# QueensGambit/CrazyAra

Hardware: AMD Instinct MI355X
Metric: nn_evals_per_sec (higher is better)
Workload: dtype f16x3; 1 GPU; crazyhouse RISEv2 19-block (34x8x8 planes -> 5184 policy + value), batch=256, inputs resident in HBM, random-init seeded weights; batch=256, parallelism=replicas x1, precision=float16x3

## Files before the change

crazyara_amd/csrc/nn/kernels.h:

```cpp
#pragma once
#include <hip/hip_runtime.h>
#include <cstdint>

namespace cra {

typedef _Float16 half_t;

constexpr int kSquares = 64;

inline int64_t packed_weight_elems(int cout_pad, int k_total) { return int64_t(cout_pad) * k_total; }

struct ConvArgs {
    const void* x;
    const void* wpk;
    const void* wpk_lo;
    const float* bias;
    const void* resid;
    void* out;
    int batch;
    int cin;
    int cout_pad;
    int cout_real;
    int cout_ld;
    int ks;
// ... 13 lines not shown
    float pre_acc_scale;
    int dev;
    int few_boards;
    int x_ld;
};

template <typename T> void launch_conv_gemm(const ConvArgs& a, hipStream_t s);

struct BlockArgs {
    const void* x;
    void* y;
    const void* w1pk;
    const float* b1;
    const float* wdw;
    const float* b2;
    const void* w3pk;
    const void* w1pk_lo;
    const void* w3pk_lo;
    const float* b3;
    int batch, C, cop_pad, ks;
    const float* gate;
    float* pool_out;
    const float* dwpk;
};
template <typename T> void launch_block(const BlockArgs& a, hipStream_t s);
void launch_conv_gemm_x3(const ConvArgs& a, hipStream_t s);
void launch_block_x3(const BlockArgs& a, hipStream_t s);
void init_x3_kernel_attributes();
int block_x3_chunk_channels();
struct X3TowerBlock {
    const void *w1pk, *w1pk_lo, *w3pk, *w3pk_lo;
    const float* dwpk;
    const float* b3;
    const float* se_w1t;
    const float* se_w2t;
    const float* se_b;
    int cop_pad;
    int se_kind;
    float w1_inv, w3_scale, w3_inv;
    int tail;
};
static_assert(sizeof(X3TowerBlock) == 96, "the tower kernels index a device array of these");
struct X3TowerArgs {
    const float* x;
    float* y;
    const X3TowerBlock* blocks;
    int nblocks;
    int batch;
    int p8;
    int ks;
    int symmetric;
    int no_tail;
    int no_quad;
};
void launch_tower_x3(const X3TowerArgs& a, hipStream_t s);
const char* tower_x3_kernel_name(const X3TowerArgs& a);
void launch_tower_x3_tail(const X3TowerArgs& a, hipStream_t s);
void init_x3_tail_kernel_attributes();
void launch_tower_x3_quad(const X3TowerArgs& a, hipStream_t s);
void init_x3_quad_kernel_attributes();
bool block_x3w_supports(int C, int ks);
void launch_block_x3w(const BlockArgs& a, hipStream_t s);
void init_x3_wblock_kernel_attributes();
void launch_se_gate_w(const float* pool, float* gate, int kind, const float* w1t, const float* w2t, const float* b1, int batch, int C, hipStream_t s);
constexpr int kX3WSplitMaxG = 8;
struct X3WSplitArgs {
    BlockArgs blk;
    const float* x_parts;
    float* y_parts;
    int gin, G;
    int stream_in;
};
int x3w_split_chunks(int cop_pad);
int x3w_split_shares(int cop_pad, int boards, int cu_count);
void launch_block_x3w_split(const X3WSplitArgs& a, hipStream_t s);
void launch_x3w_split_finish(const float* parts, int gin, float* y, float* pool_out, int batch, int C, hipStream_t s);
void init_x3_wsplit_kernel_attributes();
struct X3WTowerBlock {
    const void *w1pk, *w1pk_lo, *w3pk, *w3pk_lo;
    const float* dwpk;
    const float* b3;
    int cop_pad, ks;
};
static_assert(sizeof(X3WTowerBlock) == 56, "tower_x3w_kernel indexes a device array of these");
struct X3WTowerArgs {
    const float* x;
    float* y;
    const X3WTowerBlock* blocks;
    int nblocks;
    const float* gate;
    float* pool_out;
    int batch, C;
};
bool tower_x3w_supports(int C, int ks);
void launch_tower_x3w(const X3WTowerArgs& a, hipStream_t s);
void init_x3_wtower_kernel_attributes();
struct NtbLayer {
    const void *wh, *wl;
    const float* bias;
};
struct NtbArgs {
    const float* x;
    float* y;
    int batch, C, D, M, H;
    NtbLayer patch, qkv, proj, projection, mhca, mhca_proj, mlp1, mlp2;
};
// ... 194 lines not shown
```

crazyara_amd/csrc/nn/precision.cpp:

```cpp
#include <cstdlib>
#include <stdexcept>

#include "rise_net.h"

namespace cra {

namespace {
constexpr bool kX3ValueHeadOneLaunch = true;
}

RiseNet::DevSwitches::DevSwitches() {
    if (const char* e = getenv("CRA_X3_CONV_DEV")) conv_dev = atoi(e);
    device_graph = getenv("CRA_DEVICE_GRAPH") != nullptr;
    lane_graph = getenv("CRA_LANE_GRAPH") != nullptr;
    lane_no_graph = getenv("CRA_LANE_NO_GRAPH") != nullptr;
    predict_copy = getenv("CRA_PREDICT_COPY") != nullptr;
    predict_zero_copy = getenv("CRA_PREDICT_ZERO_COPY") != nullptr;
    if (const char* e = getenv("CRA_LANE_LAUNCHES")) lane_launches = e[0];
    lane_sync = getenv("CRA_LANE_SYNC") != nullptr;
    if (const char* e = getenv("CRA_X3_TOWER")) x3_symmetric = e[0] == 's';
    if (const char* e = getenv("CRA_X3_SPLIT_DEV")) x3_split_dev = atoi(e);
    no_small_path = getenv("CRA_NO_SMALL_PATH") != nullptr;
    if (const char* e = getenv("CRA_SMALL_BATCH_CONV_SPLIT")) small_conv_split = atoi(e);
    tower_trace = getenv("CRA_TOWER_TRACE") != nullptr;
    x3_value_one_launch = kX3ValueHeadOneLaunch;
    if (const char* e = getenv("CRA_X3_VALUE_HEAD")) x3_value_one_launch = e[0] == 'o';
    value_head_debug = getenv("CRA_VALUE_HEAD_DEBUG") != nullptr;
    if (const char* e = getenv("CRA_VALUE_HEAD_LDS_PAD")) value_head_lds_pad = atoi(e);
    if (const char* e = getenv("CRA_VALUE_HEAD_VARIANT")) value_head_variant = atoi(e);
    x3_no_head_chain = getenv("CRA_X3_NO_HEAD_CHAIN") != nullptr;
    x3_no_tail = getenv("CRA_X3_NO_TAIL") != nullptr;
    x3_no_quad = getenv("CRA_X3_NO_QUAD") != nullptr;
    small_batch_heads_apart = getenv("CRA_SMALL_BATCH_HEADS_APART") != nullptr;
}

Precision parse_precision(const std::string& precision) {
    Precision v;
    std::string prec = precision;
    auto strip = [&](const std::string& tag) {
        if (prec.size() <= tag.size() || prec.compare(prec.size() - tag.size(), tag.size(), tag) != 0) return false;
        prec.resize(prec.size() - tag.size());
        return true;
    };
    if (strip("-3k")) v.one_launch = false;
    if (strip("-8w")) v.thin_waves = true;
    if (strip("-1wg")) v.board_split = false;
    if (strip("-1b")) v.boards_per_wg = 1;
    else if (strip("-2b")) v.boards_per_wg = 2;
    if (strip("-wtower")) v.wtower = v.wnet = v.wblock = true;
    else if (strip("-wsplit")) v.wsplit = v.wnet = v.wblock = true;
    else if (strip("-wnet")) v.wnet = v.wblock = true;
    else if (strip("-wblock")) v.wblock = true;
    if (strip("-unfused")) v.fused = v.tower = false;
    else if (strip("-perblock")) v.tower = false;
    using M = Precision::Mode;
    static const std::pair<const char*, M> kModes[] = {
        {"float16", M::Float16},   {"fp16", M::Float16},     {"half", M::Float16},      {"int8", M::Int8},
        {"fp8", M::Fp8},           {"float8", M::Fp8},       {"float32", M::Float32},   {"fp32", M::Float32},
        {"float16x3", M::Float16x3}, {"fp16x3", M::Float16x3}, {"f16x3", M::Float16x3},
        {"float16p8", M::Float16p8}, {"fp16p8", M::Float16p8}, {"f16p8", M::Float16p8}};
    for (const auto& m : kModes)
        if (prec == m.first) {
            v.mode = m.second;
            if (v.wtower && !v.x3()) throw std::invalid_argument("`-wtower` is a float16x3 kernel family (float16x3-wtower | float16p8-wtower), got '" + precision + "'");
            if (v.wtower && !v.fused) throw std::invalid_argument("`-wtower` and `-unfused` exclude each other, got '" + precision + "'");
            if (v.wsplit && !v.x3()) throw std::invalid_argument("`-wsplit` is a float16x3 kernel family (float16x3-wsplit | float16p8-wsplit), got '" + precision + "'");
            if (v.wsplit && !v.fused) throw std::invalid_argument("`-wsplit` and `-unfused` exclude each other, got '" + precision + "'");
            if (v.wsplit && !v.board_split)
                throw std::invalid_argument("`-wsplit` and `-1wg` exclude each other (several workgroups per board against one), got '" + precision + "'");
            if (v.wnet && !v.x3()) throw std::invalid_argument("`-wnet` is a float16x3 kernel family (float16x3-wnet | float16p8-wnet), got '" + precision + "'");
            if (v.wnet && !v.fused) throw std::invalid_argument("`-wnet` and `-unfused` exclude each other, got '" + precision + "'");
            if (v.wblock && !v.x3()) throw std::invalid_argument("`-wblock` is a float16x3 kernel family (float16x3-wblock | float16p8-wblock), got '" + precision + "'");
            if (v.wblock && !v.fused) throw std::invalid_argument("`-wblock` and `-unfused` exclude each other, got '" + precision + "'");
            return v;
        }
    throw std::invalid_argument("unsupported precision '" + precision + "' (float16 | float16x3 | float16p8 | float32 | fp8 | int8)");
}

}
```

crazyara_amd/csrc/nn/rise_net.h:

```cpp
#pragma once
#include <hip/hip_runtime.h>
#include <memory>
#include <string>
#include <utility>
#include <vector>

#include "board_net.h"
#include "netfile.h"

namespace cra {

uint8_t float_to_e4m3(float v);
uint8_t float_to_e5m2(float v);

struct Precision {
    enum class Mode { Float32, Float16, Float16x3, Float16p8, Fp8, Int8 };
    Mode mode = Mode::Float16;
    bool fused = true;
    bool tower = true;
    bool one_launch = true;
    bool thin_waves = false;
    bool board_split = true;
    bool wblock = false;
    bool wnet = false;
// ... 57 lines not shown
    void time_ops(int iters, float* ms);
    float time_forward(int iters);

    struct IoOverride {
        const float* planes = nullptr;
        float* value = nullptr;
        float* probs = nullptr;
        float* aux = nullptr;
    };
    bool last_submit_was_zero_copy() const { return last_zero_copy_; }

private:
    friend class ExpertSet;
    struct ForwardCall {
        int boards = 0;
        const IoOverride* io = nullptr;
        int prev_g = 1;
    };
    RiseNet(const std::string& model_path, int device_id, int batch_size, const std::string& precision, const RiseNet* parent);
    struct Impl;
    template <typename T> struct Builder;
    template <typename T> void build(const NetFile& nf);
    template <typename T> void enqueue(hipStream_t s, ForwardCall call);
    template <typename T> void launch_op(int i, hipStream_t s, ForwardCall& call);
    void launch_forward_in_stream(ForwardCall call);
    void forward_on(hipStream_t s, ForwardCall call);
    int boards_of_call(int n_valid) const;
    void capture();
    bool buffers_are_pinned(const float* in_planes, float* value, float* probs, float* aux);
    bool last_zero_copy_ = false;
    bool counted_in_flight_ = false;
    int staged_calls_left_ = 0;
    struct DevSwitches {
        int conv_dev = -1;
        bool device_graph = false;
        bool lane_graph = false;
        bool lane_no_graph = false;
        bool predict_copy = false;
        bool predict_zero_copy = false;
        char lane_launches = 0;
        bool lane_sync = false;
        bool x3_symmetric = false;
        int x3_split_dev = 0;
        bool no_small_path = false;
        int small_conv_split = 2;
        bool tower_trace = false;
        bool x3_value_one_launch;
        bool value_head_debug = false;
        int value_head_lds_pad = -1;
        int value_head_variant = 0;
        bool x3_no_head_chain = false;
        bool x3_no_tail = false;
        bool x3_no_quad = false;
        bool small_batch_heads_apart = false;
        DevSwitches();
    } dev_;
    float* value_head_dbg_ = nullptr;

    std::string model_file_path_;
    Precision prec_;
    std::vector<std::pair<float, float>> int8_calib_;
    static constexpr int kBoardSplitMaxBatch = 64;
    std::unique_ptr<RiseNet> small_;
    bool owns_stream_ = true;
    int stream_slot_ = -1;
    std::string precision_arg_;
    int cu_count_ = 256;
    int launches_ = 0;
    hipGraph_t graph_ = nullptr;
    hipGraphExec_t graph_exec_ = nullptr;
    void* d_desc_ = nullptr;
    std::unique_ptr<Impl> impl_;
};

std::string int8_calibration_path(const std::string& model_file_path);
std::vector<std::pair<float, float>> read_int8_calibration(const std::string& model_file_path);
std::string calibrate_int8(const std::string& model_path, int device_id, const float* planes_host, int n_boards);
std::vector<float> default_calibration_planes(int channels, int version, int* n_boards);

}
```

crazyara_amd/csrc/nn/rise_net_build.hip:

```cpp
#include <algorithm>
#include <cmath>
#include <cstring>
#include <type_traits>

#include "../chess/planes_host.h"
#include "pack.h"
#include "rise_net_impl.h"

namespace cra {

namespace {
enum class Family {
    Tower,
    X3Tower,
    X3Split,
    Fused,
    WBlock,
    WSplit,
    WTower,
    Layers,
    Transformer,
    WNtb
};
struct BlockPlan {
// ... 675 lines not shown
    prod_op = int(im.ops.size());
    im.ops.push_back(op);
    tower_blocks.clear();
    tower_gate = nullptr;
    std::swap(cur, nxt);
}

template <typename T> void RiseNet::Builder<T>::flush_x3_run() {
    if (x3_blocks.empty()) return;
    if (x3_split && x3_run_ks == 3) {
        if (!split_parts[0])
            for (auto& q : split_parts) q = static_cast<float*>(im.dalloc(size_t(B) * kSplitMaxG * kSquares * C * sizeof(float)));
        const int max_g = std::max(1, std::min(int(kSplitMaxG), net.cu_count_ / B));
        const int nb = int(x3_blocks.size());
        int gin = 1;
        for (int k = 0; k < nb; ++k) {
            Op op;
            op.kind = OpKind::BlockX3Split;
            op.xs.blk = x3_blocks[k];
            op.xs.x_parts = k == 0 ? reinterpret_cast<const float*>(cur) : split_parts[k % 2];
            op.xs.y_parts = split_parts[(k + 1) % 2];
            op.xs.gin = gin;
            op.xs.batch = B;
            op.xs.G = std::min(max_g, x3_blocks[k].cop_pad / block_x3_chunk_channels());
            op.xs.dev = dev.x3_split_dev;
            if (k > 0 && x3_blocks[k].se_kind != 0 && !(dev.x3_split_dev & 8)) {
                float* pools = static_cast<float*>(im.dalloc(size_t(B) * kSplitMaxG * C * sizeof(float)));
                im.ops.back().xs.pool_out = pools;
                op.xs.pool_in = pools;
            }
            gin = op.xs.G;
            im.ops.push_back(op);
        }
        Op fin;
        fin.kind = OpKind::X3SplitFinish;
        fin.xs.x_parts = split_parts[nb % 2];
        fin.xs.gin = gin;
        fin.xs.batch = B;
        fin.xs_y = reinterpret_cast<float*>(nxt);
        im.ops.push_back(fin);
    } else {
        Op op;
        op.kind = OpKind::TowerX3;
        op.tx.x = reinterpret_cast<const float*>(cur);
        op.tx.y = reinterpret_cast<float*>(nxt);
        op.tx.blocks = im.upload(x3_blocks);
        op.tx.nblocks = int(x3_blocks.size());
        op.tx.batch = B;
        op.tx.p8 = prec.p8() ? 1 : 0;
        op.tx.ks = x3_run_ks;
        op.tx.symmetric = dev.x3_symmetric ? 1 : 0;
        op.tx.no_tail = dev.x3_no_tail ? 1 : 0;
        op.tx.no_quad = dev.x3_no_quad ? 1 : 0;
        im.ops.push_back(op);
    }
    x3_blocks.clear();
    prod_op = -1;
    std::swap(cur, nxt);
}

template <typename T> void RiseNet::Builder<T>::one_launch_head() {
    const Folded fv = fold_bn(nf, "value_head.body.0", "value_head.body.1");
    const HeadStreams hs = pack_head(fold_bn(nf, "policy_head.body.0", "policy_head.body.1"), fold_bn(nf, "policy_head.body.3", ""), fv, C, cv, cp);
    Op op;
    op.kind = OpKind::Head;
    HeadArgs& h = op.hd;
    h.x = cur;
    h.logits = net.d_logits_;
    h.probs = net.d_probs_;
    h.value = net.d_value_;
    h.aux = net.d_aux_;
    h.s1 = im.upload(hs.s1);
    h.b1 = im.upload(hs.b1);
    h.s2 = im.upload(hs.s2);
    h.s1_wave_frags = 9 * 16 + 16 + 16;
    h.s2_wave_frags = 18 * 3 + 9;
    h.vconv_bias = im.upload_d2f(fv.b, 8);
    h.cp = cp;
    h.batch = B;
    if (dev.tower_trace) h.trace = static_cast<unsigned long long*>(im.dalloc(64 * sizeof(unsigned long long)));
    const int nfl = kSquares * cv;
    if (wdl) {
        h.fc1_w = im.upload(pack_value_wdl(nf, nfl, 512));
        const float* bw = nf.get("value_head.body_wdl.0.bias").data;
        h.wdl_b[0] = bw[0]; h.wdl_b[1] = bw[1]; h.wdl_b[2] = bw[2];
        h.wdl_b[3] = nf.get("value_head.body_plys.0.bias").data[0];
        h.wdlp = 1;
        macs += 4.0 * nfl;
    } else {
        const TensorView& w2 = nf.get("value_head.body_final.2.weight");
        const float* bb = nf.get("value_head.body_final.0.bias").data;
        h.fc1_w = im.upload(pack_value_fc1_threads(nf, nfl, fc));
        h.fc1_b = im.upload(std::vector<float>(bb, bb + fc));
        h.fc2_w = im.upload(std::vector<float>(w2.data, w2.data + fc));
        h.fc2_b = nf.get("value_head.body_final.2.bias").data[0];
        macs += double(nfl) * fc + fc;
    }
    macs += double(kSquares) * 9 * (double(C) * C + double(C) * cp) + double(kSquares) * C * cv;
    im.ops.push_back(op);
}

template <typename T> void RiseNet::Builder<T>::policy_head() {
    const bool head_chain = prec.p8() && policy_map && C == 256 && round_up(cp, 16) <= 128 && !x3_split;
    const bool head_chain_x3 = prec.x3() && !prec.p8() && prec.fused && policy_map && C == 256 && round_up(cp, 16) <= 128 && !x3_split &&
                               !dev.x3_no_head_chain;
    if (head_chain || head_chain_x3) {
// ... 207 lines not shown
```

crazyara_amd/csrc/nn/x3.hip:

```cpp
#include "kernels.h"
#include "device_utils.h"
#include "value_head_body.h"
#include "x3_device.h"

#include <algorithm>
#include <cstdlib>
#include <stdexcept>
#include <type_traits>

#ifndef X3_SGB_VALU
#define X3_SGB_VALU 10
#endif

namespace cra {

namespace {

typedef int i32x4_x3 __attribute__((ext_vector_type(4)));
typedef int i32x8_x3 __attribute__((ext_vector_type(8)));
__device__ __forceinline__ uint32_t x3_high_bytes(uint32_t p01, uint32_t p23) {
    return __builtin_amdgcn_perm(p23, p01, 0x07050301u);
}
__device__ __forceinline__ void split4_b8(const float (&v)[4], half4& hi, uint32_t& h8, uint32_t& l8) {
    uint32_t h[2], l[2];
// ... 1943 lines not shown
            *reinterpret_cast<f32x4*>(yb + size_t(x3_square(t * 16 + l15)) * C + (w * NJ + j) * 16 + lg * 4) = accX[j][t];
}

void init_x3_kernel_attributes() {
    (void)hipFuncSetAttribute(reinterpret_cast<const void*>(&block_x3_kernel), hipFuncAttributeMaxDynamicSharedMemorySize, int(X3Block::lds_bytes));
    (void)hipFuncSetAttribute(reinterpret_cast<const void*>(&tower_x3_kernel), hipFuncAttributeMaxDynamicSharedMemorySize, int(X3Block::lds_bytes));
    (void)hipFuncSetAttribute(reinterpret_cast<const void*>(&block_x3_split_kernel), hipFuncAttributeMaxDynamicSharedMemorySize, int(X3Block::lds_bytes));
    (void)hipFuncSetAttribute(reinterpret_cast<const void*>(&tower_x3_roles_kernel<3>), hipFuncAttributeMaxDynamicSharedMemorySize, int(X3Block::lds_bytes));
    (void)hipFuncSetAttribute(reinterpret_cast<const void*>(&tower_x3_roles_kernel<5>), hipFuncAttributeMaxDynamicSharedMemorySize, int(X3Block::lds_bytes + 8192));
    init_x3_tail_kernel_attributes();
    init_x3_quad_kernel_attributes();
    (void)hipFuncSetAttribute(reinterpret_cast<const void*>(&tower_p8_kernel<3>), hipFuncAttributeMaxDynamicSharedMemorySize, int(X3Block::lds_bytes));
    (void)hipFuncSetAttribute(reinterpret_cast<const void*>(&tower_p8_kernel<5>), hipFuncAttributeMaxDynamicSharedMemorySize, int(X3Block::lds_bytes + 8192));
    (void)hipFuncSetAttribute(reinterpret_cast<const void*>(&conv3x3_x3_chain_kernel), hipFuncAttributeMaxDynamicSharedMemorySize, int(ConvX3::lds_bytes));
    const int conv_p8_lds = int(ConvP8::lds_bytes);
    (void)hipFuncSetAttribute(reinterpret_cast<const void*>(&conv3x3_p8_chain_kernel), hipFuncAttributeMaxDynamicSharedMemorySize, conv_p8_lds);
    (void)hipFuncSetAttribute(reinterpret_cast<const void*>(&conv3x3_p8_kernel<2, 8>), hipFuncAttributeMaxDynamicSharedMemorySize, conv_p8_lds);
    (void)hipFuncSetAttribute(reinterpret_cast<const void*>(&conv3x3_p8_kernel<1, 8>), hipFuncAttributeMaxDynamicSharedMemorySize, conv_p8_lds);
}
int block_x3_chunk_channels() { return X3Block::CK; }

void launch_block_x3(const BlockArgs& a, hipStream_t s) {
    hipLaunchKernelGGL(block_x3_kernel, dim3(a.batch), dim3(X3Block::NTHR), X3Block::lds_bytes, s, a);
}
void launch_block_x3_split(const X3SplitArgs& a, hipStream_t s) {
    const int n = a.blk.cop_pad / X3Block::CK;
    if (a.G < 1 || a.G > n || a.G > 16 || a.gin < 1 || a.gin > 16) throw std::invalid_argument("block_x3_split: 1 <= G <= min(chunks, 16), 1 <= gin <= 16");
    hipLaunchKernelGGL(block_x3_split_kernel, dim3(8 * a.G * ((a.batch + 7) / 8)), dim3(X3Block::NTHR), X3Block::lds_bytes, s, a);
}
void launch_x3_split_finish(const float* parts, int gin, float* y, int batch, hipStream_t s) {
    const int n4 = batch * 64 * X3Block::C / 4;
    hipLaunchKernelGGL(x3_split_finish_kernel, dim3(std::min(1024, (n4 + 255) / 256)), dim3(256), 0, s, parts, gin, y, batch);
}
namespace {
enum class X3TowerKernel { P8_5, P8_3, Quad3, Tail5, Tail3, Roles5, Roles3, Symmetric };
X3TowerKernel pick_tower_x3(const X3TowerArgs& a) {
    const bool symmetric = a.symmetric != 0;
    if (a.p8) {
        if (symmetric) throw std::invalid_argument("Precision float16p8 runs the two-role tower only");
        return a.ks == 5 ? X3TowerKernel::P8_5 : X3TowerKernel::P8_3;
    }
    if (!symmetric && !a.no_tail) {
        if (a.ks == 5) return X3TowerKernel::Tail5;
        return a.no_quad ? X3TowerKernel::Tail3 : X3TowerKernel::Quad3;
    }
    if (a.ks == 5) return X3TowerKernel::Roles5;
    return symmetric ? X3TowerKernel::Symmetric : X3TowerKernel::Roles3;
}
}
const char* tower_x3_kernel_name(const X3TowerArgs& a) {
    switch (pick_tower_x3(a)) {
        case X3TowerKernel::P8_5: return "tower_p8_kernel<5>";
        case X3TowerKernel::P8_3: return "tower_p8_kernel<3>";
        case X3TowerKernel::Quad3: return "tower_x3_quad_kernel<3>";
        case X3TowerKernel::Tail5: return "tower_x3_tail_kernel<5>";
        case X3TowerKernel::Tail3: return "tower_x3_tail_kernel<3>";
        case X3TowerKernel::Roles5: return "tower_x3_roles_kernel<5>";
        case X3TowerKernel::Roles3: return "tower_x3_roles_kernel<3>";
        case X3TowerKernel::Symmetric: return "tower_x3_kernel";
    }
    return "?";
}
void launch_tower_x3(const X3TowerArgs& a, hipStream_t s) {
    switch (pick_tower_x3(a)) {
        case X3TowerKernel::P8_5: hipLaunchKernelGGL(tower_p8_kernel<5>, dim3(a.batch), dim3(X3Block::NTHR), X3Block::lds_bytes + 8192, s, a); break;
        case X3TowerKernel::P8_3: hipLaunchKernelGGL(tower_p8_kernel<3>, dim3(a.batch), dim3(X3Block::NTHR), X3Block::lds_bytes, s, a); break;
        case X3TowerKernel::Quad3: launch_tower_x3_quad(a, s); break;
        case X3TowerKernel::Tail5:
        case X3TowerKernel::Tail3: launch_tower_x3_tail(a, s); break;
        case X3TowerKernel::Roles5: hipLaunchKernelGGL(tower_x3_roles_kernel<5>, dim3(a.batch), dim3(X3Block::NTHR), X3Block::lds_bytes + 8192, s, a); break;
        case X3TowerKernel::Roles3: hipLaunchKernelGGL(tower_x3_roles_kernel<3>, dim3(a.batch), dim3(X3Block::NTHR), X3Block::lds_bytes, s, a); break;
        case X3TowerKernel::Symmetric: hipLaunchKernelGGL(tower_x3_kernel, dim3(a.batch), dim3(X3Block::NTHR), X3Block::lds_bytes, s, a); break;
    }
}

}
```

crazyara_amd/csrc/nn/x3_quad.cpp:

```cpp
#include "x3_device.h"
#include "x3_quad.h"

#include <type_traits>

namespace cra {

template <int KS>
__global__ __launch_bounds__(512) void tower_x3_quad_kernel(const X3TowerArgs a) {
    static_assert(KS == 3, "depthwise 3x3 (X3DepthwiseQuad); 5x5 runs stay on tower_x3_tail_kernel");
    constexpr int REC = 256;
    using G = X3Block;
    static_assert(G::NE == 1 && G::T2BUF == 2 && G::CK == 128, "the role kernel uses the NE = 1 tile geometry (two t2 buffers of 128 channels)");
    static_assert(X3Q_T2T_HALVES <= 64 * G::TROW, "t2T of a chunk lies in the [64][TROW] tile's place");
    constexpr int C = G::C, CK = G::CK, XROW = G::XROW, TROW = G::TROW;
    extern __shared__ __attribute__((aligned(16))) char smem[];
    const X3Tiles T = x3_tiles(smem);
    const int b = blockIdx.x;
    const int tid = threadIdx.x, lane = tid & 63, l15 = lane & 15, lg = lane >> 4;
    const int wave = __builtin_amdgcn_readfirstlane(tid >> 6);
    const bool expand_role = wave < 4;
    const int w = wave & 3;
    const uint32_t lane_off = uint32_t(lane) * 16u;
    x3_stage_tile(T, a.x + size_t(b) * 64 * C, nullptr, tid);
    __syncthreads();
    constexpr int EW = 2;
    half8 e_h[EW][2], e_l[EW][2];
    bool first_chunk_requested = false;
    if (expand_role) {
    for (int blk = 0; blk < a.nblocks; ++blk) {
        const X3TowerBlock& d = a.blocks[blk];
        if (blk > 0 && d.se_kind != 0) {
            x3_se_gate_from_mean(d, reinterpret_cast<float*>(T.t2h), tid);
            __syncthreads();
            first_chunk_requested = false;
#pragma unroll
            for (int ne = 0; ne < 2; ++ne) {
#pragma unroll
                for (int q = 0; q < EW; ++q) { asm volatile("" : "=v"(e_h[q][ne])); asm volatile("" : "=v"(e_l[q][ne])); }
            }
        }
        const X3Weights W = x3_weights(d.w1pk, d.w1pk_lo, d.w3pk, d.w3pk_lo, d.dwpk, d.cop_pad);
        const int n = W.cop_pad / CK;
        const bool tail = __builtin_amdgcn_readfirstlane(d.tail) != 0;
#ifdef CRA_X3_TRACE
        const bool tracing = (b == 0 || b == 131) && blk == CRA_X3_TRACE;
        int trace_n = 0;
#endif
        {
            const X3QuadOffsets qo = x3_quad_offsets(lane);
            int sto[4];
#pragma unroll
            for (int t = 0; t < 4; ++t) sto[t] = x3q_store_offset(0, l15, lg, t);
            auto e_tile = [&](int i, int ne) { return i * (CK / 16) + (tail && i == n - 1 ? w : w * 2 + ne); };
            auto load_e = [&](auto one_c, int i, int s) {
                if constexpr (X3_ABL & 16) return;
#pragma unroll
                for (int ne = 0; ne < (decltype(one_c)::value ? 1 : 2); ++ne) {
                    const uint32_t f = uint32_t(e_tile(i, ne)) * (C / 32) + uint32_t(s);
                    e_h[s % EW][ne] = x3_frag(W.w1h, lane_off, f);
                    e_l[s % EW][ne] = x3_frag(W.w1l, lane_off, f);
                }
            };
            auto load_first_chunk = [&](const X3Weights& Wx, bool one) {
                if constexpr (X3_ABL & 16) return;
#pragma unroll
                for (int s = 0; s < EW; ++s)
#pragma unroll
                    for (int ne = 0; ne < 2; ++ne) {
                        const uint32_t f = uint32_t(one ? w : w * 2 + ne) * (C / 32) + uint32_t(s);
                        e_h[s][ne] = x3_frag(Wx.w1h, lane_off, f);
                        e_l[s][ne] = x3_frag(Wx.w1l, lane_off, f);
                    }
            };
            if constexpr (X3_ABL & 16) {
#pragma unroll
                for (int s = 0; s < EW; ++s)
#pragma unroll
                    for (int ne = 0; ne < 2; ++ne) e_h[s][ne] = e_l[s][ne] = *reinterpret_cast<const half8*>(T.xh + lane * 8);
            }
            if (!first_chunk_requested) load_first_chunk(W, tail && n == 1);
            float* const my_dws = T.dws + (w * 2) * REC;
            f32x4 accE[2][4], accD[2][4];
            X3DepthwiseQuad dw;
            auto interval = [&](auto hase_c, auto hasd_c, auto onee_c, auto oned_c, int i) {
                constexpr bool HASE = decltype(hase_c)::value, HASD = decltype(hasd_c)::value;
                constexpr bool ONEE = decltype(onee_c)::value, ONED = decltype(oned_c)::value;
                static_assert(!(ONEE && !HASE) && !(ONED && (HASE || !HASD)), "the tail chunk is expanded in interval n - 1 and runs the depthwise alone in interval n");
                constexpr int NEE = ONEE ? 1 : 2;
                half8 ring_h[4], ring_l[4];
                auto read_step = [&](int st) {
                    if constexpr (X3_ABL & 8) {
                        ring_h[st % 4] = e_h[0][0];
                        ring_l[st % 4] = e_l[0][0];
                    } else {
                        ring_h[st % 4] = *reinterpret_cast<const half8*>(T.xh + ((st & 3) * 16 + l15) * XROW + (st >> 2) * 32 + lg * 8);
                        ring_l[st % 4] = *reinterpret_cast<const half8*>(T.xl + ((st & 3) * 16 + l15) * XROW + (st >> 2) * 32 + lg * 8);
                    }
                };
                f32x4 dw_raw[NEE][REC / 256];
                if constexpr (HASE) {
// ... 47 lines not shown
                                if constexpr (X3_ABL & 64) {
                                    asm volatile("" ::"v"(h), "v"(l));
                                } else {
                                    *reinterpret_cast<half4*>(t2h + tile * 16 * X3Q_T2T_ROW + sto[t]) = h;
                                    *reinterpret_cast<half4*>(t2l + tile * 16 * X3Q_T2T_ROW + sto[t]) = l;
                                }
                            }
                        }
                    }
                    if constexpr (HASE && HASD) {
#pragma unroll
                        for (int r = 0; r < 12 * NEE; ++r) {
                            __builtin_amdgcn_sched_group_barrier(0x008, 1, 0);
                            __builtin_amdgcn_sched_group_barrier(0x002, ONEE ? 8 : 4, 0);
                        }
                    }
                    __builtin_amdgcn_sched_barrier(0);
                }
                if constexpr (HASE) {
#pragma unroll
                    for (int ne = 0; ne < NEE; ++ne)
#pragma unroll
                        for (int h2 = 0; h2 < REC / 256; ++h2) *reinterpret_cast<f32x4*>(my_dws + ne * REC + h2 * 256 + lane * 4) = dw_raw[ne][h2];
#pragma unroll
                    for (int ne = 0; ne < NEE; ++ne)
#pragma unroll
                        for (int t = 0; t < 4; ++t) accD[ne][t] = accE[ne][t];
                }
            };
            constexpr std::true_type yes{};
            constexpr std::false_type no{};
            auto run = [&](auto hase_c, auto hasd_c, auto onee_c, auto oned_c, int i) {
                const int kk = i - 1;
                X3_STAMP(0);
                interval(hase_c, hasd_c, onee_c, oned_c, i);
                X3_STAMP(3);
                if constexpr (!(X3_ABL & 32)) __syncthreads();
                X3_STAMP(4);
            };
            const int nfull = tail ? n - 1 : n;
            if (nfull == 0) run(yes, no, yes, no, 0);
            else run(yes, no, no, no, 0);
            for (int i = 1; i < nfull; ++i) run(yes, yes, no, no, i);
            if (tail) {
                if (nfull > 0) run(yes, yes, yes, no, n - 1);
                run(no, yes, no, yes, n);
            } else run(no, yes, no, no, n);
            first_chunk_requested = false;
            if (blk + 1 < a.nblocks && a.blocks[blk + 1].se_kind == 0) {
                const X3TowerBlock& dn = a.blocks[blk + 1];
                load_first_chunk(x3_weights(dn.w1pk, dn.w1pk_lo, dn.w3pk, dn.w3pk_lo, dn.dwpk, dn.cop_pad), dn.tail != 0 && dn.cop_pad == CK);
                first_chunk_requested = true;
            }
            __syncthreads();
            { const int kk = n; X3_STAMP(5); }
        }
    }
    } else {
    constexpr int NJ = 4;
    f32x4 accX[NJ][4];
    x3_stream_load<NJ>(accX, a.x + size_t(b) * 64 * C, w * NJ, l15, lg);
    for (int blk = 0; blk < a.nblocks; ++blk) {
        const X3TowerBlock& d = a.blocks[blk];
        if (blk > 0 && d.se_kind != 0) x3_stream_se<NJ>(T, d, accX, reinterpret_cast<float*>(T.t2h), w * NJ, tid);
        const X3Weights W = x3_weights(d.w1pk, d.w1pk_lo, d.w3pk, d.w3pk_lo, d.dwpk, d.cop_pad);
        const int n = W.cop_pad / CK;
        const int nslab3 = W.cop_pad >> 5;
        const bool tail = __builtin_amdgcn_readfirstlane(d.tail) != 0;
#ifdef CRA_X3_TRACE
        const bool tracing = (b == 0 || b == 131) && blk == CRA_X3_TRACE;
        int trace_n = 0;
#endif
        {
            constexpr int PW = 2;
            half8 p_h[PW][NJ], p_l[PW][NJ];
            int rdo[2][4];
#pragma unroll
            for (int hh = 0; hh < 2; ++hh)
#pragma unroll
                for (int t = 0; t < 4; ++t) rdo[hh][t] = x3q_read_offset(0, hh, t, l15, lg);
            auto load_p = [&](int k, int s2) {
                if constexpr (X3_ABL & 16) return;
#pragma unroll
                for (int j = 0; j < NJ; ++j) {
                    const uint32_t f = uint32_t(w * NJ + j) * uint32_t(nslab3) + uint32_t(k * (CK / 32) + s2);
                    p_h[s2 % PW][j] = x3_frag(W.w3h, lane_off, f);
                    p_l[s2 % PW][j] = x3_frag(W.w3l, lane_off, f);
                }
            };
            if constexpr (X3_ABL & 16) {
#pragma unroll
                for (int s2 = 0; s2 < PW; ++s2)
#pragma unroll
                    for (int j = 0; j < NJ; ++j) p_h[s2][j] = p_l[s2][j] = *reinterpret_cast<const half8*>(T.xl + lane * 8);
            }
            x3_stream_add_bias<NJ>(accX, d.b3, w * NJ, lg);
#pragma unroll
            for (int s2 = 0; s2 < PW; ++s2) load_p(0, s2);
            if constexpr (!(X3_ABL & 32)) {
                __syncthreads();
                __syncthreads();
            }
            auto project = [&](auto one_c, int kk) {
                constexpr int NS2 = decltype(one_c)::value ? CK / 64 : CK / 32;
                const half_t* const t2h = T.t2h + (kk & 1) * 64 * TROW;
                const half_t* const t2l = T.t2l + (kk & 1) * 64 * TROW;
                const half_t* rd[2][4];
#pragma unroll
                for (int hh = 0; hh < 2; ++hh)
#pragma unroll
                    for (int t = 0; t < 4; ++t) rd[hh][t] = t2h + rdo[hh][t];
                const int to_lo = int(t2l - t2h);
                X3_STAMP(8);
                half8 bh[2][4], bl[2][4];
                auto read_t2 = [&](int s2, half8 (&h)[4], half8 (&l)[4]) {
#pragma unroll
                    for (int t = 0; t < 4; ++t) {
                        if constexpr (X3_ABL & 8) {
                            h[t] = p_h[s2 % PW][0];
                            l[t] = p_l[s2 % PW][0];
                        } else {
                            h[t] = x3q_read_fragment(rd[0][t] + s2 * 32 * X3Q_T2T_ROW, rd[1][t] + s2 * 32 * X3Q_T2T_ROW);
                            l[t] = x3q_read_fragment(rd[0][t] + s2 * 32 * X3Q_T2T_ROW + to_lo, rd[1][t] + s2 * 32 * X3Q_T2T_ROW + to_lo);
                        }
                    }
                };
                read_t2(0, bh[0], bl[0]);
#pragma unroll
                for (int s2 = 0; s2 < NS2; ++s2) {
                    if (s2 + 1 < NS2) read_t2(s2 + 1, bh[(s2 + 1) & 1], bl[(s2 + 1) & 1]);
                    __builtin_amdgcn_sched_barrier(0);
#pragma unroll
                    for (int j = 0; j < NJ; ++j)
#pragma unroll
                        for (int t = 0; t < 4; ++t) x3_mfma(p_l[s2 % PW][j], bh[s2 & 1][t], accX[j][t], !(X3_ABL & 4));
#pragma unroll
                    for (int j = 0; j < NJ; ++j)
#pragma unroll
                        for (int t = 0; t < 4; ++t) x3_mfma(p_h[s2 % PW][j], bl[s2 & 1][t], accX[j][t], !(X3_ABL & 4));
#pragma unroll
                    for (int j = 0; j < NJ; ++j)
#pragma unroll
                        for (int t = 0; t < 4; ++t) x3_mfma(p_h[s2 % PW][j], bh[s2 & 1][t], accX[j][t], !(X3_ABL & 4));
                    if (s2 + PW < NS2) load_p(kk, s2 + PW);
                    else if constexpr (decltype(one_c)::value) load_p(kk, s2 + PW - NS2);
                    else load_p(kk + 1 < n ? kk + 1 : kk, s2 + PW - NS2);
                    if (s2 == 1) X3_STAMP(9);
                    __builtin_amdgcn_sched_barrier(0);
                }
                X3_STAMP(10);
            };
            const int nfull = tail ? n - 1 : n;
            for (int kk = 0; kk < nfull; ++kk) {
                project(std::false_type{}, kk);
                if (kk + 1 < n) {
                    if constexpr (!(X3_ABL & 32)) __syncthreads();
                }
                X3_STAMP(11);
            }
            if (tail) {
                const int kk = n - 1;
                project(std::true_type{}, kk);
                X3_STAMP(11);
            }
            if (blk + 1 < a.nblocks && a.blocks[blk + 1].se_kind == 0) x3_stream_write_tiles<NJ>(T, accX, w * NJ, l15, lg);
            { const int kk = n; X3_STAMP(12); }
            __syncthreads();
            { const int kk = n; X3_STAMP(13); }
        }
    }
    x3_stream_store<NJ>(accX, a.y + size_t(b) * 64 * C, w * NJ, l15, lg);
    }
}

void init_x3_quad_kernel_attributes() {
    (void)hipFuncSetAttribute(reinterpret_cast<const void*>(&tower_x3_quad_kernel<3>), hipFuncAttributeMaxDynamicSharedMemorySize, int(X3Block::lds_bytes));
}
void launch_tower_x3_quad(const X3TowerArgs& a, hipStream_t s) {
    hipLaunchKernelGGL(tower_x3_quad_kernel<3>, dim3(a.batch), dim3(X3Block::NTHR), X3Block::lds_bytes, s, a);
}

}
```

crazyara_amd/csrc/nn/x3_quad.h:

```cpp
#pragma once

namespace cra {

constexpr int x3q_row(int sq) { return ((sq >> 3) & 3) * 16 + (sq >> 5) * 8 + (sq & 7); }
constexpr int x3q_square(int row) { return ((row >> 4) + 4 * ((row >> 3) & 1)) * 8 + (row & 7); }
constexpr int x3q_lane_square(int t, int lg, int r) { return (4 * (lg >> 1) + t) * 8 + 4 * (lg & 1) + r; }

constexpr int X3Q_T2T_ROW = 64;
constexpr int X3Q_T2T_HALVES = 128 * X3Q_T2T_ROW;
constexpr int x3q_swizzle(int c) { return (c & 1) | (((c >> 2) & 1) << 1) | (((c >> 1) & 1) << 2) | (c & 8); }
constexpr int x3q_t2t_offset(int c, int row) { return c * X3Q_T2T_ROW + 4 * ((row >> 2) ^ x3q_swizzle(c & 15)) + (row & 3); }
constexpr int x3q_store_offset(int tile, int l15, int lg, int t) { return x3q_t2t_offset(tile * 16 + l15, t * 16 + 4 * lg); }
constexpr int x3q_read_offset(int s2, int hh, int t, int l15, int lg) { return x3q_t2t_offset(s2 * 32 + lg * 8 + hh * 4 + (l15 >> 2), t * 16 + 4 * (l15 & 3)); }

}

#ifdef __HIPCC__
namespace cra {
namespace {

struct X3QuadOffsets {
    int hl, hr;
    int vt, vt6;
    int vb2, vb;
    int k0, k6, k2, k8;
    int to_v, to_k;
};
__device__ __forceinline__ X3QuadOffsets x3_quad_offsets(int lane) {
    const int lg = lane >> 4;
    const bool odd = (lg & 1) != 0, hi = lg >= 2;
    X3QuadOffsets o;
    o.hl = odd ? 0 : 11 * 16;
    o.hr = odd ? 5 * 16 : 0;
    o.vt = hi ? 0 : 11 * 16;
    o.vt6 = hi ? 0 : 5 * 16;
    o.vb2 = hi ? 11 * 16 : 0;
    o.vb = hi ? 6 * 16 : 0;
    o.k0 = lg == 3 ? 0 : 11 * 16;
    o.k6 = lg == 2 ? 0 : 5 * 16;
    o.k2 = lg == 1 ? 0 : 11 * 16;
    o.k8 = lg == 0 ? 0 : 5 * 16;
    o.to_v = (lane ^ 32) * 4;
    o.to_k = (lane ^ 48) * 4;
    return o;
}

struct X3DepthwiseQuad {
    float w[11];
    float whl[3], whr[3];
    float wvt[3], wvb[3];
    float wk[4];
    float S[4][4], H[4], V[4], K;
    float outv[4][4];

    __device__ __forceinline__ void load(const float* rec, int l15, const X3QuadOffsets& o) {
        const float* p = rec + l15;
#pragma unroll
        for (int q = 0; q < 11; ++q) w[q] = p[q * 16];
#pragma unroll
        for (int d = 0; d < 3; ++d) {
            whl[d] = p[o.hl + d * 16];
            whr[d] = p[o.hr + (6 + d) * 16];
            wvt[d] = p[(d == 2 ? o.vt6 : o.vt) + 3 * d * 16];
            wvb[d] = p[(d == 0 ? o.vb2 : o.vb) + (3 * d + 2) * 16];
        }
        wk[0] = p[o.k0];
// ... 9 lines not shown
        if constexpr (X3_ABL & 1) return;
        const bool odd = (lg & 1) != 0, hi = lg >= 2;
        float sh[4];
#pragma unroll
        for (int t = 0; t < 4; ++t) {
            sh[t] = odd ? S[t][0] : S[t][3];
            H[t] = __builtin_bit_cast(float, __builtin_amdgcn_ds_swizzle(__builtin_bit_cast(int, sh[t]), 0x401f));
        }
#pragma unroll
        for (int r = 0; r < 4; ++r) {
            const float sv = hi ? S[0][r] : S[3][r];
            V[r] = __builtin_bit_cast(float, __builtin_amdgcn_ds_bpermute(o.to_v, __builtin_bit_cast(int, sv)));
        }
        const float sk = hi ? sh[0] : sh[3];
        K = __builtin_bit_cast(float, __builtin_amdgcn_ds_bpermute(o.to_k, __builtin_bit_cast(int, sk)));
    }
    template <int Y, int X, int Q> __device__ __forceinline__ float tap(float a) const {
        constexpr int DX = Q / 3, DY = Q % 3;
        if constexpr (Y >= 0 && Y < 4 && X >= 0 && X < 4) return fmaf(w[Q], S[Y][X], a);
        else if constexpr (Y >= 0 && Y < 4) return fmaf(X < 0 ? whl[DY] : whr[DY], H[Y], a);
        else if constexpr (X >= 0 && X < 4) return fmaf(Y < 0 ? wvt[DX] : wvb[DX], V[X], a);
        else return fmaf(wk[(Y < 0 ? 0 : 2) + (X < 0 ? 0 : 1)], K, a);
    }
    template <int T, int R> __device__ __forceinline__ void output() {
        if constexpr (X3_ABL & 1) {
            outv[T][R] = S[T][R];
            return;
        }
        float a = w[10];
        a = tap<T - 1, R - 1, 0>(a); a = tap<T - 1, R, 3>(a); a = tap<T - 1, R + 1, 6>(a);
        a = tap<T, R - 1, 1>(a);     a = tap<T, R, 4>(a);     a = tap<T, R + 1, 7>(a);
        a = tap<T + 1, R - 1, 2>(a); a = tap<T + 1, R, 5>(a); a = tap<T + 1, R + 1, 8>(a);
        outv[T][R] = fmaxf(a, 0.f);
    }
    template <int T> __device__ __forceinline__ void taps_rank() {
        output<T, 0>(); output<T, 1>(); output<T, 2>(); output<T, 3>();
    }
    template <int T> __device__ __forceinline__ void pin_rank() {
#pragma unroll
        for (int r = 0; r < 4; ++r) asm volatile("" : "+v"(outv[T][r]));
    }
};

typedef __fp16 x3q_f16x4 __attribute__((__vector_size__(4 * sizeof(__fp16))));
__device__ __forceinline__ half8 x3q_read_fragment(const half_t* lo4, const half_t* hi4) {
    typedef __attribute__((address_space(3))) x3q_f16x4 lds_f16x4;
    typedef uint32_t u32x2 __attribute__((ext_vector_type(2)));
    typedef uint32_t u32x4 __attribute__((ext_vector_type(4)));
    const u32x2 a = __builtin_bit_cast(u32x2, __builtin_amdgcn_ds_read_tr16_b64_v4f16((lds_f16x4*)(lo4)));
    const u32x2 b = __builtin_bit_cast(u32x2, __builtin_amdgcn_ds_read_tr16_b64_v4f16((lds_f16x4*)(hi4)));
    return __builtin_bit_cast(half8, u32x4{a.x, a.y, b.x, b.y});
}

}
}
#endif
```

Baseline: 353,600 evals/s.

## Prefetch SE gate weights early and park them in LDS for the quad tower

For squeeze-excitation blocks of kind 1, the expand-role waves now request the next block's SE FC weights during the previous block's tail. Part of the first FC matrix is parked in the xh/xl LDS tiles for the stream-role waves, and the expand role computes the FCs there directly. The stream role's SE step reads the parked weights from LDS instead of global memory, aiming to hide gate-weight load latency behind the previous block's work. The old behaviour stays behind a CRA_X3_LATE_GATE switch. This adds extra barriers, register pressure from 48 f32x4 weight registers, and reuse of LDS that must not clash with the tiles.

```diff
diff --git a/crazyara_amd/csrc/nn/kernels.h b/crazyara_amd/csrc/nn/kernels.h
--- a/crazyara_amd/csrc/nn/kernels.h
+++ b/crazyara_amd/csrc/nn/kernels.h
@@ -89,6 +89,7 @@
     int symmetric;
     int no_tail;
     int no_quad;
+    int late_gate;
 };
 void launch_tower_x3(const X3TowerArgs& a, hipStream_t s);
 const char* tower_x3_kernel_name(const X3TowerArgs& a);
diff --git a/crazyara_amd/csrc/nn/precision.cpp b/crazyara_amd/csrc/nn/precision.cpp
--- a/crazyara_amd/csrc/nn/precision.cpp
+++ b/crazyara_amd/csrc/nn/precision.cpp
@@ -31,6 +31,7 @@
     x3_no_head_chain = getenv("CRA_X3_NO_HEAD_CHAIN") != nullptr;
     x3_no_tail = getenv("CRA_X3_NO_TAIL") != nullptr;
     x3_no_quad = getenv("CRA_X3_NO_QUAD") != nullptr;
+    x3_late_gate = getenv("CRA_X3_LATE_GATE") != nullptr;
     small_batch_heads_apart = getenv("CRA_SMALL_BATCH_HEADS_APART") != nullptr;
 }
 
diff --git a/crazyara_amd/csrc/nn/rise_net.h b/crazyara_amd/csrc/nn/rise_net.h
--- a/crazyara_amd/csrc/nn/rise_net.h
+++ b/crazyara_amd/csrc/nn/rise_net.h
@@ -133,6 +133,7 @@
         bool x3_no_head_chain = false;
         bool x3_no_tail = false;
         bool x3_no_quad = false;
+        bool x3_late_gate = false;
         bool small_batch_heads_apart = false;
         DevSwitches();
     } dev_;
diff --git a/crazyara_amd/csrc/nn/rise_net_build.hip b/crazyara_amd/csrc/nn/rise_net_build.hip
--- a/crazyara_amd/csrc/nn/rise_net_build.hip
+++ b/crazyara_amd/csrc/nn/rise_net_build.hip
@@ -751,6 +751,7 @@
         op.tx.symmetric = dev.x3_symmetric ? 1 : 0;
         op.tx.no_tail = dev.x3_no_tail ? 1 : 0;
         op.tx.no_quad = dev.x3_no_quad ? 1 : 0;
+        op.tx.late_gate = dev.x3_late_gate ? 1 : 0;
         im.ops.push_back(op);
     }
     x3_blocks.clear();
diff --git a/crazyara_amd/csrc/nn/x3.hip b/crazyara_amd/csrc/nn/x3.hip
--- a/crazyara_amd/csrc/nn/x3.hip
+++ b/crazyara_amd/csrc/nn/x3.hip
@@ -2019,7 +2019,7 @@
     switch (pick_tower_x3(a)) {
         case X3TowerKernel::P8_5: return "tower_p8_kernel<5>";
         case X3TowerKernel::P8_3: return "tower_p8_kernel<3>";
-        case X3TowerKernel::Quad3: return "tower_x3_quad_kernel<3>";
+        case X3TowerKernel::Quad3: return a.late_gate ? "tower_x3_quad_kernel<3, late gate>" : "tower_x3_quad_kernel<3>";
         case X3TowerKernel::Tail5: return "tower_x3_tail_kernel<5>";
         case X3TowerKernel::Tail3: return "tower_x3_tail_kernel<3>";
         case X3TowerKernel::Roles5: return "tower_x3_roles_kernel<5>";
diff --git a/crazyara_amd/csrc/nn/x3_quad.cpp b/crazyara_amd/csrc/nn/x3_quad.cpp
--- a/crazyara_amd/csrc/nn/x3_quad.cpp
+++ b/crazyara_amd/csrc/nn/x3_quad.cpp
@@ -5,7 +5,10 @@
 
 namespace cra {
 
-template <int KS>
+static_assert(X3Q_PARK_BYTES <= int(2 * 64 * X3Block::XROW * sizeof(half_t)), "the parked gate matrix lies in xh + xl");
+constexpr int X3Q_TRACE_GATE = 13;
+
+template <int KS, bool LATE_GATE = false>
 __global__ __launch_bounds__(512) void tower_x3_quad_kernel(const X3TowerArgs a) {
     static_assert(KS == 3, "depthwise 3x3 (X3DepthwiseQuad); 5x5 runs stay on tower_x3_tail_kernel");
     constexpr int REC = 256;
@@ -27,11 +30,38 @@
     half8 e_h[EW][2], e_l[EW][2];
     bool first_chunk_requested = false;
     if (expand_role) {
+#ifdef CRA_X3_TRACE
+    int trace_n = 0;
+#endif
     for (int blk = 0; blk < a.nblocks; ++blk) {
         const X3TowerBlock& d = a.blocks[blk];
-        if (blk > 0 && d.se_kind != 0) {
+#ifdef CRA_X3_TRACE
+        const bool tracing = (b == 0 || b == 131) && blk == CRA_X3_TRACE;
+#endif
+        if (blk > 0 && d.se_kind != 0 && (LATE_GATE || d.se_kind != 1)) {
+#ifdef CRA_X3_TRACE
+            {
+                constexpr int kk = X3Q_TRACE_GATE;
+                f32x4 wa[16], wb[16];
+#pragma unroll
+                for (int i = 0; i < 16; ++i) wa[i] = reinterpret_cast<const f32x4*>(d.se_w1t)[i * 512 + tid];
+#pragma unroll
+                for (int i = 0; i < 16; ++i) wb[i] = reinterpret_cast<const f32x4*>(d.se_kind == 1 ? d.se_w2t : d.se_w1t + size_t(16) * 512 * 4)[i * 512 + tid];
+                X3_STAMP(0);
+#pragma unroll
+                for (int i = 0; i < 16; ++i) { asm volatile("s_waitcnt vmcnt(0)" : "+v"(wa[i]), "+v"(wb[i])); }
+                X3_STAMP(1);
+                __syncthreads();
+                X3_STAMP(2);
+                x3_se_fcs(d, reinterpret_cast<float*>(T.t2h), reinterpret_cast<float*>(T.t2h) + 8 * 36, reinterpret_cast<float*>(T.t2h) + 12 * 36, wa, wb, tid);
+                X3_STAMP(3);
+                __syncthreads();
+                X3_STAMP(4);
+            }
+#else
             x3_se_gate_from_mean(d, reinterpret_cast<float*>(T.t2h), tid);
             __syncthreads();
+#endif
             first_chunk_requested = false;
 #pragma unroll
             for (int ne = 0; ne < 2; ++ne) {
@@ -42,10 +72,6 @@
         const X3Weights W = x3_weights(d.w1pk, d.w1pk_lo, d.w3pk, d.w3pk_lo, d.dwpk, d.cop_pad);
         const int n = W.cop_pad / CK;
         const bool tail = __builtin_amdgcn_readfirstlane(d.tail) != 0;
-#ifdef CRA_X3_TRACE
-        const bool tracing = (b == 0 || b == 131) && blk == CRA_X3_TRACE;
-        int trace_n = 0;
-#endif
         {
             const X3QuadOffsets qo = x3_quad_offsets(lane);
             int sto[4];
@@ -199,25 +225,59 @@
                 load_first_chunk(x3_weights(dn.w1pk, dn.w1pk_lo, dn.w3pk, dn.w3pk_lo, dn.dwpk, dn.cop_pad), dn.tail != 0 && dn.cop_pad == CK);
                 first_chunk_requested = true;
             }
-            __syncthreads();
-            { const int kk = n; X3_STAMP(5); }
+            if (!LATE_GATE && blk + 1 < a.nblocks && a.blocks[blk + 1].se_kind == 1) {
+                const X3TowerBlock& dn = a.blocks[blk + 1];
+#ifdef CRA_X3_TRACE
+                const bool tracing = (b == 0 || b == 131) && blk + 1 == CRA_X3_TRACE;
+                constexpr int kk = X3Q_TRACE_GATE;
+#endif
+                f32x4 wa[16], wb[16];
+                x3q_gate_request(dn, reinterpret_cast<f32x4*>(T.xh), wa, wb, tid);
+                X3_STAMP(0);
+#ifdef CRA_X3_TRACE
+#pragma unroll
+                for (int i = 0; i < 16; ++i) { asm volatile("s_waitcnt vmcnt(0)" : "+v"(wa[i]), "+v"(wb[i])); }
+                X3_STAMP(1);
+#endif
+                __syncthreads();
+                X3_STAMP(5);
+                __syncthreads();
+                X3_STAMP(2);
+                float* const scratch = reinterpret_cast<float*>(T.t2h);
+                x3_se_fcs(dn, scratch, scratch + 8 * 36, scratch + 12 * 36, wa, wb, tid);
+                X3_STAMP(3);
+                load_first_chunk(x3_weights(dn.w1pk, dn.w1pk_lo, dn.w3pk, dn.w3pk_lo, dn.dwpk, dn.cop_pad), dn.tail != 0 && dn.cop_pad == CK);
+                first_chunk_requested = true;
+                __syncthreads();
+                X3_STAMP(4);
+            } else {
+                __syncthreads();
+                { const int kk = n; X3_STAMP(5); }
+            }
         }
     }
     } else {
     constexpr int NJ = 4;
     f32x4 accX[NJ][4];
     x3_stream_load<NJ>(accX, a.x + size_t(b) * 64 * C, w * NJ, l15, lg);
+#ifdef CRA_X3_TRACE
+    int trace_n = 0;
+#endif
     for (int blk = 0; blk < a.nblocks; ++blk) {
         const X3TowerBlock& d = a.blocks[blk];
-        if (blk > 0 && d.se_kind != 0) x3_stream_se<NJ>(T, d, accX, reinterpret_cast<float*>(T.t2h), w * NJ, tid);
+#ifdef CRA_X3_TRACE
+        const bool tracing = (b == 0 || b == 131) && blk == CRA_X3_TRACE;
+#endif
+        if (blk > 0 && d.se_kind != 0) {
+            { [[maybe_unused]] constexpr int kk = X3Q_TRACE_GATE; X3_STAMP(8); }
+            if (!LATE_GATE && d.se_kind == 1) x3q_stream_se_parked<NJ>(T, d, accX, reinterpret_cast<float*>(T.t2h), reinterpret_cast<const f32x4*>(T.xh), w * NJ, tid);
+            else x3_stream_se<NJ>(T, d, accX, reinterpret_cast<float*>(T.t2h), w * NJ, tid);
+            { [[maybe_unused]] constexpr int kk = X3Q_TRACE_GATE; X3_STAMP(12); }
+        }
         const X3Weights W = x3_weights(d.w1pk, d.w1pk_lo, d.w3pk, d.w3pk_lo, d.dwpk, d.cop_pad);
         const int n = W.cop_pad / CK;
         const int nslab3 = W.cop_pad >> 5;
         const bool tail = __builtin_amdgcn_readfirstlane(d.tail) != 0;
-#ifdef CRA_X3_TRACE
-        const bool tracing = (b == 0 || b == 131) && blk == CRA_X3_TRACE;
-        int trace_n = 0;
-#endif
         {
             constexpr int PW = 2;
             half8 p_h[PW][NJ], p_l[PW][NJ];
@@ -322,9 +382,11 @@
 
 void init_x3_quad_kernel_attributes() {
     (void)hipFuncSetAttribute(reinterpret_cast<const void*>(&tower_x3_quad_kernel<3>), hipFuncAttributeMaxDynamicSharedMemorySize, int(X3Block::lds_bytes));
+    (void)hipFuncSetAttribute(reinterpret_cast<const void*>(&tower_x3_quad_kernel<3, true>), hipFuncAttributeMaxDynamicSharedMemorySize, int(X3Block::lds_bytes));
 }
 void launch_tower_x3_quad(const X3TowerArgs& a, hipStream_t s) {
-    hipLaunchKernelGGL(tower_x3_quad_kernel<3>, dim3(a.batch), dim3(X3Block::NTHR), X3Block::lds_bytes, s, a);
+    if (a.late_gate) hipLaunchKernelGGL((tower_x3_quad_kernel<3, true>), dim3(a.batch), dim3(X3Block::NTHR), X3Block::lds_bytes, s, a);
+    else hipLaunchKernelGGL(tower_x3_quad_kernel<3>, dim3(a.batch), dim3(X3Block::NTHR), X3Block::lds_bytes, s, a);
 }
 
 }
diff --git a/crazyara_amd/csrc/nn/x3_quad.h b/crazyara_amd/csrc/nn/x3_quad.h
--- a/crazyara_amd/csrc/nn/x3_quad.h
+++ b/crazyara_amd/csrc/nn/x3_quad.h
@@ -12,6 +12,11 @@
 constexpr int x3q_t2t_offset(int c, int row) { return c * X3Q_T2T_ROW + 4 * ((row >> 2) ^ x3q_swizzle(c & 15)) + (row & 3); }
 constexpr int x3q_store_offset(int tile, int l15, int lg, int t) { return x3q_t2t_offset(tile * 16 + l15, t * 16 + 4 * lg); }
 constexpr int x3q_read_offset(int s2, int hh, int t, int l15, int lg) { return x3q_t2t_offset(s2 * 32 + lg * 8 + hh * 4 + (l15 >> 2), t * 16 + 4 * (l15 & 3)); }
+
+constexpr int X3Q_PARK_THREADS = 256;
+constexpr int X3Q_PARK_BYTES = 16 * X3Q_PARK_THREADS * 16;
+constexpr int x3q_park_index(int i, int p) { return i * X3Q_PARK_THREADS + p; }
+constexpr int x3q_park_source(int i, int p) { return i * 512 + X3Q_PARK_THREADS + p; }
 
 }
 
@@ -127,6 +132,65 @@
     return __builtin_bit_cast(half8, u32x4{a.x, a.y, b.x, b.y});
 }
 
+__device__ __forceinline__ f32x4 x3q_load_f32x4(__amdgpu_buffer_rsrc_t r, uint32_t lane_off, uint32_t off) {
+    return __builtin_bit_cast(f32x4, __builtin_amdgcn_raw_buffer_load_b128(r, lane_off, off, 0));
+}
+__device__ __forceinline__ void x3q_gate_request(const X3TowerBlock& d, f32x4* park, f32x4 (&wa)[16], f32x4 (&wb)[16], int p) {
+    const __amdgpu_buffer_rsrc_t w1 = x3_rsrc(d.se_w1t), w2 = x3_rsrc(d.se_w2t);
+    const uint32_t off = uint32_t(p) * 16u;
+    f32x4 wp[16];
+#pragma unroll
+    for (int i = 0; i < 16; ++i) wp[i] = x3q_load_f32x4(w1, off, uint32_t(x3q_park_source(i, 0)) * 16u);
+#pragma unroll
+    for (int i = 0; i < 16; ++i) wa[i] = x3q_load_f32x4(w1, off, uint32_t(i * 512) * 16u);
+#pragma unroll
+    for (int i = 0; i < 16; ++i) wb[i] = x3q_load_f32x4(w2, off, uint32_t(i * 512) * 16u);
+#pragma unroll
+    for (int i = 0; i < 16; ++i) park[x3q_park_index(i, p)] = wp[i];
+}
+template <int NJ>
+__device__ __forceinline__ void x3q_stream_se_parked(const X3Tiles& T, const X3TowerBlock& d, f32x4 (&x)[NJ][4], float* scratch, const f32x4* park, int tile0, int tid) {
+    constexpr int GRP = 36;
+    const int lane = tid & 63, l15 = lane & 15, lg = lane >> 4;
+    f32x4 wa[16], wb[16];
+    {
+        const __amdgpu_buffer_rsrc_t w2 = x3_rsrc(d.se_w2t);
+#pragma unroll
+        for (int i = 0; i < 16; ++i) wb[i] = x3q_load_f32x4(w2, uint32_t(tid) * 16u, uint32_t(i * 512) * 16u);
+    }
+#pragma unroll
+    for (int j = 0; j < NJ; ++j) {
+        float sum[4];
+#pragma unroll
+        for (int r = 0; r < 4; ++r) sum[r] = (x[j][0][r] + x[j][1][r]) + (x[j][2][r] + x[j][3][r]);
+#pragma unroll
+        for (int r = 0; r < 4; ++r) {
+            sum[r] += dpp_mov<0x111>(sum[r]);
+            sum[r] += dpp_mov<0x112>(sum[r]);
+            sum[r] += dpp_mov<0x114>(sum[r]);
+            sum[r] += dpp_mov<0x118>(sum[r]);
+        }
+        if (l15 == 15) {
+            const int c = (tile0 + j) * 16 + lg * 4;
+#pragma unroll
+            for (int r = 0; r < 4; ++r) scratch[((c + r) >> 5) * GRP + ((c + r) & 31)] = sum[r] * (1.f / 64.f);
+        }
+    }
+#pragma unroll
+    for (int i = 0; i < 16; ++i) wa[i] = park[x3q_park_index(i, tid - X3Q_PARK_THREADS)];
+    __syncthreads();
+    x3_se_fcs(d, scratch, scratch + 8 * GRP, scratch + 12 * GRP, wa, wb, tid);
+    const float* se_gate = scratch + 12 * GRP;
+#pragma unroll
+    for (int j = 0; j < NJ; ++j) {
+        const f32x4 g = *reinterpret_cast<const f32x4*>(se_gate + (tile0 + j) * 16 + lg * 4);
+#pragma unroll
+        for (int t = 0; t < 4; ++t) x[j][t] *= g;
+    }
+    x3_stream_write_tiles<NJ>(T, x, tile0, l15, lg);
+    __syncthreads();
+}
+
 }
 }
 #endif
```

Result: no change. 353,900 evals/s (median of 3 runs) (+0.1%).
